# anuradhawick/kmertools

Hardware: AMD Instinct MI355X
Metric: Gbases/s on comp-oligo k=4 and ctr k=31, 150bp synthetic reads, 1/2/4/8 GPU (higher is better)
Workload: dtype f64

## Files before the change

kmertools_amd/csrc/kt_bulk.hip:

```cpp
#include <stdio.h>
#include <stdlib.h>

#include <new>
#include <type_traits>
#include <vector>

#include "kt_launch.hpp"
#include "kt_segment.hpp"
#include "kt_superkmer.hpp"
#include "kt_table.hpp"

namespace {

using ktseg::SegArgs;
using ktseg::SegShared;
using kttab::Slot;
using kttab::TableRef;

constexpr int BLOCK = ktseg::BLOCK;
#ifndef KT_BUILD_T
#define KT_BUILD_T 1024
#endif
#ifndef KT_ABLATION
#define KT_ABLATION 0
#endif
constexpr uint32_t LOG2_S = kttab::LOG2_RANGE;
constexpr uint32_t S = 1u << LOG2_S;
constexpr uint32_t MAX_B = 2048;
#ifndef KT_STORE_HASH
#define KT_STORE_HASH 1
#endif
#ifndef KT_P2_BIG32_PER
#define KT_P2_BIG32_PER 16
#endif
#ifndef KT_P2_T64
#define KT_P2_T64 512
#endif
template <class K, bool BIG>
constexpr int p2t() { return BIG ? (sizeof(K) == 8 ? KT_P2_T64 : 1024) : 512; }
template <class K, bool BIG>
constexpr bool p2_sdig() { return !BIG && !(sizeof(K) == 8 && KT_STORE_HASH); }
template <class K, bool BIG>
constexpr uint32_t chunk2() { return sizeof(K) == 8 ? (BIG ? 16384u : 8192u) : (BIG ? (uint32_t)KT_P2_BIG32_PER : 32u) * p2t<K, BIG>(); }

struct Plan {
    uint32_t n;
    uint32_t m8;
    uint32_t b1, b2;
    uint32_t B1, B2;
    uint32_t G;
    uint64_t cap1;
    uint64_t cap2;
    uint64_t room1;
    uint32_t nxs, xmap;
    uint32_t dbg;
    uint32_t lists;
    uint32_t kbits;
};

template <class K>
constexpr K empty_of() { return (K) ~(K)0; }

struct Meta {
    uint32_t *H;
    uint64_t *O;
    uint64_t *bstart;
    uint64_t *gcur;
    unsigned long long *dump;
    unsigned long long *xcur;
    uint32_t *ovf;
    kt_seg_src *srcs;
    uint32_t *fail;
    uint64_t *fstart;
    uint64_t *fend;
    uint64_t *spill_n;
    uint64_t *spill_keys;
    uint32_t *spill_counts;
    uint64_t spill_cap;
};

__device__ __forceinline__ uint32_t digit1h(uint64_t h, const Plan &p) { return (uint32_t)(h >> 32) >> (32 - p.b1); }
__device__ __forceinline__ uint32_t digit2h(uint64_t h, const Plan &p) {
    return ((uint32_t)(h >> 32) >> (32 - p.b1 - p.b2)) & (p.B2 - 1);
}
__device__ __forceinline__ uint32_t digit1(uint64_t key, const Plan &p) { return digit1h(ktd::khash_k(key, p.kbits), p); }
static_assert(KT_KHASH == 1 || !KT_STORE_HASH,
              "the empty marker must not be the hash of a k-mer (true for the multiplicative hash)");
template <class K>
constexpr bool stores_hash() { return sizeof(K) == 8 && KT_STORE_HASH; }
template <class K>
// ... 1485 lines not shown
            for (uint32_t i = tid; i < B2; i += P2T) {
                fstart[(uint64_t)jl * B2 + i] = lo + (uint64_t)i * cap2;
                fend[(uint64_t)jl * B2 + i] = lo + sm.cur[i];
            }
        } else if (tid == 0) {
            fail[jl] = 1u;
            atomicAdd(&fail[p.B1], 1u);
        }
        ktd::lds_barrier();
    }
}

template <class K>
struct SwwcShared {
    K *buf;
    uint32_t *fc;
    uint32_t *flags;
    static size_t bytes(uint32_t B2) { return (size_t)B2 * 128 + (size_t)B2 * 8 + 64; }
    __device__ SwwcShared(unsigned char *raw, uint32_t B2) {
        buf = reinterpret_cast<K *>(raw);
        fc = reinterpret_cast<uint32_t *>(raw + (size_t)B2 * 128);
        flags = fc + 2 * B2;
    }
};
#ifndef KT_SWWC_T64
#define KT_SWWC_T64 1024
#endif
#ifndef KT_SWWC_T32
#define KT_SWWC_T32 1024
#endif
template <class K>
constexpr int swwc_t() { return sizeof(K) == 8 ? KT_SWWC_T64 : KT_SWWC_T32; }

template <class K>
__global__ __launch_bounds__((swwc_t<K>()), (swwc_t<K>() / 256)) void part2_swwc_kernel(P2In in, Plan p, K *__restrict__ keys2,
                                                              uint64_t *__restrict__ fstart, uint64_t *__restrict__ fend,
                                                              uint32_t *__restrict__ fail) {
    extern __shared__ __attribute__((aligned(16))) unsigned char smem_raw[];
    const SwwcShared<K> sm(smem_raw, p.B2);
    constexpr K EMPTY = empty_of<K>();
#ifndef KT_SWWC_PER32
#define KT_SWWC_PER32 16
#endif
#ifndef KT_SWWC_PER64
#define KT_SWWC_PER64 8
#endif
    constexpr int P2T = swwc_t<K>(), PER = sizeof(K) == 8 ? KT_SWWC_PER64 : KT_SWWC_PER32 * 512 / P2T;
    constexpr uint32_t CH = (uint32_t)P2T * PER;
    constexpr uint32_t LK = 128 / sizeof(K), LSH = sizeof(K) == 8 ? 4 : 5;
    constexpr uint32_t GL = 8;
    constexpr uint32_t KPL = LK / GL;
    const uint32_t tid = threadIdx.x;
    const uint32_t nd = p.B1;
    const uint32_t B2 = p.B2, cap2 = (uint32_t)p.cap2, dshift = 32 - p.b1 - p.b2;
    auto digit = [&](K stored) -> uint32_t { return ((uint32_t)(hash_of_stored<K>(stored, p) >> 32) >> dshift) & (B2 - 1u); };
    const uint32_t grp = tid / GL, gl = tid % GL;
    for (uint32_t jl = blockIdx.x; jl < nd; jl += gridDim.x) {
        const uint32_t n_seg = in.n_src;
        auto segment = [&](uint32_t sidx, const K *&base, uint64_t &n) {
            const kt_seg_src &q = in.srcs[sidx];
            const uint64_t c = q.counts[jl];
            base = reinterpret_cast<const K *>(q.keys) + (uint64_t)jl * q.cap1;
            n = c < q.cap1 ? c : q.cap1;
        };
        uint64_t total = 0;
        for (uint32_t sidx = 0; sidx < n_seg; sidx++) {
            const K *b;
            uint64_t n;
            segment(sidx, b, n);
            total += n;
        }
        if (fail[jl] != 0) continue;
        const uint64_t lo = in.out_of(jl, p.room1);
        for (uint32_t i = tid; i < 2 * B2; i += P2T) sm.fc[i] = 0;
        if (tid < 4) sm.flags[tid] = 0;
        ktd::lds_barrier();
        const kt_i32x4 outrs = buf_rsrc(keys2 + lo, (uint32_t)(p.room1 * sizeof(K)));
        const uint32_t allow_a = (uint32_t)__builtin_amdgcn_readfirstlane(
            (int)__float_as_uint(0.93f * (float)cap2 / (float)(total ? total : 1)));
        const uint32_t allow_b = (uint32_t)__builtin_amdgcn_readfirstlane((int)__float_as_uint(6.f * sqrtf((float)cap2) + 32.f));
        uint64_t seen = 0;
        bool failed = false;
        K kcur[PER], knext[PER];
        uint32_t qa[PER];
#ifndef KT_SWWC_FB
#define KT_SWWC_FB 4
#endif
        auto flush = [&](uint32_t g, float allowed) {
            constexpr uint32_t FB = KT_SWWC_FB, NGR = P2T / GL;
            for (uint32_t d0 = 0; d0 < B2; d0 += NGR * FB) {
                uint32_t fl[FB], cu[FB];
                bool some = false;
#pragma unroll
                for (uint32_t b = 0; b < FB; b++) {
                    const uint32_t d = d0 + b * NGR + grp;
                    fl[b] = d < B2 ? sm.fc[2 * d] : 0u;
                    cu[b] = d < B2 ? sm.fc[2 * d + 1] : 0u;
                }
#pragma unroll
                for (uint32_t b = 0; b < FB; b++) some |= (fl[b] >> LSH) != 0;
                typedef uint32_t raw4 __attribute__((ext_vector_type(4)));
                raw4 v[FB];
#pragma unroll
                for (uint32_t b = 0; b < FB; b++) v[b] = raw4{0u, 0u, 0u, 0u};
                if (__builtin_amdgcn_ballot_w64(some) != 0) {
#pragma unroll
                    for (uint32_t b = 0; b < FB; b++) {
                        const uint32_t d = d0 + b * NGR + grp;
                        v[b] = *reinterpret_cast<const raw4 *>(&sm.buf[(size_t)(d < B2 ? d : 0) * LK + gl * KPL]);
                    }
                }
#pragma unroll
                for (uint32_t b = 0; b < FB; b++) {
                    const uint32_t d = d0 + b * NGR + grp;
                    if (d0 + b * NGR >= B2) break;
                    const uint32_t fill = fl[b], cur = cu[b];
                    const bool go = (fill >> LSH) != 0;
                    const bool fits = cur + LK <= cap2;
                    const uint32_t off = go && fits ? (d * cap2 + cur + gl * KPL) * (uint32_t)sizeof(K) : BUF_DROP;
                    asm volatile("buffer_store_dwordx4 %0, %1, %2, 0 offen\n\ts_nop 1" ::"v"(v[b]), "v"(off), "s"(outrs));
                    if (go && gl == 0) {
                        sm.fc[2 * d] = fill - LK;
                        sm.fc[2 * d + 1] = cur + LK;
                        if ((fill >> LSH) > 1) sm.flags[(g + 1) & 1] = 1;
                        if (!fits || (float)(cur + fill) > allowed) sm.flags[2] = 1;
                    }
                }
            }
        };
        for (uint32_t sidx = 0; sidx < n_seg && !failed; sidx++) {
            const K *base;
            uint64_t n;
            segment(sidx, base, n);
            if (n == 0) continue;
            auto load_chunk = [&](uint64_t c0, K (&dst)[PER]) {
                const uint32_t left = (uint32_t)__builtin_amdgcn_readfirstlane((int)(n - c0 > CH ? CH : (uint32_t)(n - c0)));
                const kt_i32x4 rs = buf_rsrc(base + c0, left * (uint32_t)sizeof(K));
                uint32_t voff = tid * (uint32_t)sizeof(K);
#pragma unroll
                for (int u = 0; u < PER; u += 8) buf_load8_async<K, P2T * (int)sizeof(K)>(&dst[u], rs, voff);
            };
            load_chunk(0, knext);
            buf_take<0>(kcur, knext);
            for (uint64_t c0 = 0; c0 < n; c0 += CH) {
                uint32_t tl = tid;
                asm volatile("" : "+v"(tl));
                const uint32_t left = (uint32_t)__builtin_amdgcn_readfirstlane((int)(n - c0 > CH ? CH : (uint32_t)(n - c0)));
                if (left != CH) {
#pragma unroll
                    for (int u = 0; u < PER; u++) kcur[u] = (uint32_t)u * P2T + tl < left ? kcur[u] : EMPTY;
                }
                const bool more = c0 + CH < n;
                if (more) load_chunk(c0 + CH, knext);
                if (tl == 0) sm.flags[0] = 0;
#pragma unroll
                for (int u = 0; u < PER; u++) {
                    const uint32_t d = digit(kcur[u]);
                    const bool valid = kcur[u] != EMPTY;
                    const uint32_t q = atomicAdd(&sm.fc[2 * d], valid ? 1u : 0u);
                    qa[u] = valid ? ((q >> LSH) << 16) | (d * LK + (q & (LK - 1u))) : ~0u;
                }
                ktd::lds_barrier();
                if (sm.flags[2] != 0) {
                    failed = true;
                    if (more) buf_drain(knext);
                    break;
                }
                const uint64_t sn = seen + c0 + CH;
                const float allowed = (float)(uint32_t)(sn < total ? sn : total) * __uint_as_float(allow_a) + __uint_as_float(allow_b);
#pragma unroll
                for (int u = 0; u < PER; u++)
                    if ((qa[u] >> 16) == 0u) sm.buf[qa[u] & 0xFFFFu] = kcur[u];
                for (uint32_t i = tl; i < B2; i += P2T)
                    if ((sm.fc[2 * i] >> LSH) != 0) sm.flags[0] = 1;
                if (tl == 0) sm.flags[1] = 0;
                ktd::lds_barrier();
                bool any = sm.flags[0] != 0;
                uint32_t gens = 0;
                for (uint32_t g = 0; any; g++) {
                    flush(g, allowed);
                    gens++;
                    ktd::lds_barrier();
                    any = sm.flags[(g + 1) & 1] != 0;
                    if (tl == 0) sm.flags[g & 1] = 0;
#pragma unroll
                    for (int u = 0; u < PER; u++)
                        if ((qa[u] >> 16) == g + 1u) sm.buf[qa[u] & 0xFFFFu] = kcur[u];
                    if (any) ktd::lds_barrier();
                }
                if (more) {
                    constexpr int SPG = (1024 + P2T / GL - 1) / (P2T / GL);
                    const uint32_t issued = gens * ((B2 + P2T / GL - 1) / (P2T / GL));
                    if (issued == SPG) buf_take<SPG>(kcur, knext);
                    else if (issued == 2 * SPG) buf_take<2 * SPG>(kcur, knext);
                    else if (issued == 3 * SPG) buf_take<3 * SPG>(kcur, knext);
                    else buf_take<0>(kcur, knext);
                }
            }
            seen += n;
        }
        ktd::lds_barrier();
        if (!failed) {
            for (uint32_t d0 = 0; d0 < B2; d0 += P2T / GL) {
                const uint32_t d = d0 + grp;
                if (d >= B2) continue;
                const uint32_t fill = sm.fc[2 * d], cur = sm.fc[2 * d + 1];
                if (cur + fill > cap2) {
                    sm.flags[2] = 1;
                    continue;
                }
                for (uint32_t e = gl * KPL; e < gl * KPL + KPL; e++)
                    if (e < fill) keys2[lo + (uint64_t)d * cap2 + cur + e] = sm.buf[(size_t)d * LK + e];
                if (gl == 0) {
                    fstart[(uint64_t)jl * B2 + d] = lo + (uint64_t)d * cap2;
                    fend[(uint64_t)jl * B2 + d] = lo + (uint64_t)d * cap2 + cur + fill;
                }
            }
        }
        ktd::lds_barrier();
        if ((failed || sm.flags[2] != 0) && tid == 0) {
            fail[jl] = 1u;
            atomicAdd(&fail[p.B1], 1u);
        }
        ktd::lds_barrier();
    }
}

static_assert(LOG2_S == kttab::LOG2_RANGE, "a fine bucket is a range of the table");

constexpr int BUILD_T = KT_BUILD_T;
constexpr uint32_t LIST_CAP = 192, LIST_KEYS = LIST_CAP * (BUILD_T / 64);

template <class K>
struct lds_word;
template <>
struct lds_word<uint64_t> { using type = unsigned long long; };
template <>
struct lds_word<uint32_t> { using type = unsigned int; };

constexpr uint32_t XBLK = 8192;
static_assert(XBLK >= (1u << LOG2_S), "a range's entries fit one block");
struct ExtOut {
    uint64_t *keys;
    uint32_t *counts;
    uint64_t max;
    uint64_t *ovf_keys;
    uint32_t *ovf_counts;
    uint64_t ovf_cap;
    uint64_t *extent;
    uint32_t *fill;
    uint64_t max_blocks;
    __device__ __forceinline__ void put(uint64_t pos, uint64_t key, uint32_t occ) const {
        if (pos < max) {
            __builtin_nontemporal_store(key, keys + pos);
            __builtin_nontemporal_store(occ, counts + pos);
        } else if (pos - max < ovf_cap) {
            ovf_keys[pos - max] = key;
            ovf_counts[pos - max] = occ;
        }
    }
    __device__ __forceinline__ void get(uint64_t pos, uint64_t &key, uint32_t &occ) const {
        if (pos < max) {
            key = keys[pos];
            occ = counts[pos];
        } else {
            key = ovf_keys[pos - max];
            occ = ovf_counts[pos - max];
        }
    }
};

#ifndef KT_BUILD_DHASH
#define KT_BUILD_DHASH 1
#endif
#ifndef KT_BUILD_SGPRS
#define KT_BUILD_SGPRS 80
#endif
template <class K, bool MERGE, bool DENSE, bool EXT = false, bool DIRECT = false>
__global__ __launch_bounds__(BUILD_T) __attribute__((amdgpu_num_sgpr(KT_BUILD_SGPRS), amdgpu_waves_per_eu(8, 8))) void build_kernel(const K *__restrict__ keys2,
                                                        const uint64_t *__restrict__ fstart,
                                                        const uint64_t *__restrict__ fend, Plan p,
                                                        Slot *__restrict__ slots, uint64_t *__restrict__ spill_n,
                                                        uint64_t *__restrict__ spill_keys,
                                                        uint32_t *__restrict__ spill_counts, uint64_t spill_cap,
                                                        uint32_t *__restrict__ spill_ovf,
                                                        uint64_t *__restrict__ distinct,
                                                        uint32_t *__restrict__ range_counts, ExtOut xo) {
    static_assert(!(MERGE && DENSE), "a dense build starts from an empty table");
    static_assert(!EXT || DENSE, "only a dense build writes to the export arrays");
    static_assert(!DIRECT || (DENSE && sizeof(K) == 4), "the direct build: 32-bit keys, dense");
    extern __shared__ __attribute__((aligned(16))) unsigned char smem_raw[];
    using W = typename lds_word<K>::type;
    constexpr K EMPTY = empty_of<K>();
    const uint32_t RS = p.m8 << (LOG2_S - 3);
    K *const skeys = reinterpret_cast<K *>(smem_raw);
    uint32_t *const scounts = reinterpret_cast<uint32_t *>(smem_raw + (size_t)RS * sizeof(K));
    const uint32_t tid = threadIdx.x, lane = tid & 63u;
    const uint64_t n_fine = (uint64_t)(p.B1) * p.B2;
    const uint32_t shift = 64 - p.n;
    auto spill = [&](uint64_t key, uint32_t occurrences) {
        if (DENSE) {
            atomicOr(spill_ovf, 1u);
            return;
        }
        const uint64_t at = atomicAdd(reinterpret_cast<unsigned long long *>(spill_n), 1ull);
        if (at < spill_cap) {
            spill_keys[at] = key;
            spill_counts[at] = occurrences;
        } else {
            atomicOr(spill_ovf, 1u);
        }
    };
    __shared__ uint32_t runs[BUILD_T / 64];
    uint16_t *const mylist = reinterpret_cast<uint16_t *>(smem_raw + (size_t)RS * (sizeof(K) + 4)) + (threadIdx.x >> 6) * LIST_CAP;
    bool dirty = true;
    uint64_t xpos = 0, xend = 0;
    uint32_t xused = 0;
    long long placed = 0;
    uint64_t lo = 0, hi = 0;
    K head[4] = {EMPTY, EMPTY, EMPTY, EMPTY};
    auto load_head = [&](uint64_t l, uint64_t h, K (&dst)[4]) {
#pragma unroll
        for (int u = 0; u < 4; u++) {
            const uint64_t i = l + tid + (uint64_t)u * BUILD_T;
            dst[u] = i < h ? keys2[i] : EMPTY;
        }
    };
    if (blockIdx.x < n_fine) {
        lo = fstart[blockIdx.x];
        hi = fend[blockIdx.x];
        load_head(lo, hi, head);
    }
#if KT_ABLATION
    unsigned long long tph = __builtin_readcyclecounter();
    uint32_t phs[8] = {};
#endif
    for (uint64_t fb = blockIdx.x; fb < n_fine;) {
        const uint64_t nfb = fb + gridDim.x;
        uint64_t nlo = 0, nhi = 0;
        if (nfb < n_fine) {
            nlo = fstart[nfb];
            nhi = fend[nfb];
        }
        if (MERGE && lo == hi) {
            fb = nfb;
            lo = nlo;
            hi = nhi;
            load_head(lo, hi, head);
            continue;
        }
        if (MERGE) {
            for (uint32_t i = tid; i < RS; i += BUILD_T) {
                const uint4 v = reinterpret_cast<const uint4 *>(slots + fb * RS)[i];
                const bool occ = (v.x & v.y) != 0xFFFFFFFFu;
                skeys[i] = occ ? to_stored<K>(((uint64_t)v.y << 32) | v.x) : EMPTY;
                scounts[i] = v.z;
                placed -= occ;
            }
        } else if (dirty) {
            for (uint32_t i = tid; i < RS; i += BUILD_T) {
                if (!DIRECT) skeys[i] = EMPTY;
                scounts[i] = 0;
            }
        }
        const bool listed = !DIRECT && DENSE && p.lists != 0 && hi - lo <= LIST_KEYS && hi - lo <= RS;
        KT_PH(0);
        if (MERGE || dirty) ktd::lds_barrier();
        KT_PH(1);
        uint32_t wc = 0;
        uint32_t m0 = ~0u, m1 = ~0u;
        if constexpr (DIRECT) {
            const uint32_t sh32 = 32u - p.kbits;
            auto bump = [&](K key) {
                if (key != EMPTY) atomicAdd(&scounts[ktd::nhash((uint32_t)key, p.kbits) & (S - 1u)], 1u);
            };
            (void)sh32;
            uint64_t bbase = lo;
            for (;;) {
                const bool more = bbase + 4ull * BUILD_T < hi;
                K nxt[4] = {EMPTY, EMPTY, EMPTY, EMPTY};
                if (more) load_head(bbase + 4ull * BUILD_T, hi, nxt);
#pragma unroll
                for (int u = 0; u < 4; u++) bump(head[u]);
                if (!more) break;
                bbase += 4ull * BUILD_T;
#pragma unroll
                for (int u = 0; u < 4; u++) head[u] = nxt[u];
            }
        } else {
            constexpr bool STRIDES = KT_BUILD_DHASH && DENSE && sizeof(K) == 8;
            const uint32_t sh3 = shift - 3;
            auto hword = [&](K stored, auto hi_only) -> uint32_t {
                const uint64_t h = hash_of_stored<K>(stored, p);
                const uint32_t hi32 = (uint32_t)(h >> 32), lo32 = (uint32_t)h;
                if constexpr (decltype(hi_only)::value) return hi32 >> (sh3 - 32);
                else return __builtin_amdgcn_alignbit(hi32, lo32, sh3);
            };
            auto home_w = [&](uint32_t w) -> uint32_t { return __umul24((w >> 3) & (S - 1), p.m8) >> 3; };
            auto stride_w = [&](uint32_t w) -> uint32_t {
                if (!STRIDES) return 1u;
                return __builtin_amdgcn_perm(0x251f1d17u, 0x13110d0bu, (w & 7u) | 0x0c0c0c00u);
            };
            auto insert_batch = [&](auto chk, auto lst, auto hi_only) {
                constexpr bool CHECK = decltype(chk)::value, LISTED = decltype(lst)::value;
                K cur = head[0], q0 = head[1], q1 = head[2], q2 = LISTED ? EMPTY : head[3];
#if KT_ABLATION
                if (p.dbg & 1u) cur = EMPTY;
#endif
                uint32_t w = hword(cur, hi_only);
                uint32_t s = home_w(w), step = stride_w(w), probes = 0;
                while (cur != EMPTY) {
                    const K v = (K)atomicCAS(reinterpret_cast<W *>(&skeys[s]), (W)EMPTY, (W)cur);
                    const bool claimed = v == EMPTY, dup = v == cur;
                    bool done = claimed | dup;
                    if (dup) atomicAdd(&scounts[s], 1u);
                    if constexpr (LISTED) {
                        if (claimed) {
                            m1 = __builtin_amdgcn_alignbit(m1, m0, 16);
                            m0 = (m0 << 16) | s;
                        }
                    }
                    s += step;
                    if (s >= RS) s -= RS;
                    if (CHECK && !done && ++probes >= RS) {
                        spill(from_stored<K>(cur), 1u);
                        done = true;
                    }
                    if (done) {
                        cur = q0;
                        q0 = q1;
                        q1 = q2;
                        q2 = EMPTY;
                        w = hword(cur, hi_only);
                        s = home_w(w);
                        step = stride_w(w);
                        if (CHECK) probes = 0;
                    }
                }
            };
            const bool roomy = !MERGE && hi - lo <= RS;
            uint64_t bbase = lo;
            for (;;) {
                const bool more = bbase + 4ull * BUILD_T < hi;
                K nxt[4] = {EMPTY, EMPTY, EMPTY, EMPTY};
                if (more) load_head(bbase + 4ull * BUILD_T, hi, nxt);
                auto insert = [&](auto hi_only) {
                    if (listed) insert_batch(std::false_type{}, std::true_type{}, hi_only);
                    else if (roomy) insert_batch(std::false_type{}, std::false_type{}, hi_only);
                    else insert_batch(std::true_type{}, std::false_type{}, hi_only);
                };
                if (sh3 >= 32) insert(std::true_type{});
                else insert(std::false_type{});
                if (!more) break;
                bbase += 4ull * BUILD_T;
#pragma unroll
                for (int u = 0; u < 4; u++) head[u] = nxt[u];
            }
        }
        if (DENSE && listed) {
            const uint32_t c = (uint32_t)((m0 & 0xFFFFu) != 0xFFFFu) + (uint32_t)((m0 >> 16) != 0xFFFFu) +
                               (uint32_t)((m1 & 0xFFFFu) != 0xFFFFu);
            const uint32_t inc = wave_incl_scan(c);
            uint16_t *const at = mylist + (inc - c);
            if (c > 0) at[0] = (uint16_t)m0;
            if (c > 1) at[1] = (uint16_t)(m0 >> 16);
            if (c > 2) at[2] = (uint16_t)m1;
            wc = (uint32_t)__builtin_amdgcn_readlane((int)inc, 63);
            if (lane == 0) runs[tid >> 6] = wc;
        }
        KT_PH(2);
        ktd::lds_barrier();
        KT_PH(3);
        load_head(nlo, nhi, head);
        uint4 *dst = reinterpret_cast<uint4 *>(slots + fb * RS);
        if (DENSE) {
            constexpr uint32_t NW = BUILD_T / 64;
            const uint32_t wave = tid >> 6, share = RS / NW;
            if (!listed) {
                for (uint32_t i0 = 0; i0 < share; i0 += 64) {
                    const uint32_t i = wave * share + i0 + lane;
                    K kk;
                    uint32_t cc;
                    if constexpr (DIRECT) {
                        const uint32_t c1 = scounts[i];
                        cc = c1 - 1u;
                        kk = c1 ? (K)ktd::nhash_inv(((uint32_t)fb << LOG2_S) | i, p.kbits) : EMPTY;
                    } else {
                        kk = skeys[i];
                        cc = scounts[i];
                    }
                    const uint64_t bal = __ballot(kk != EMPTY);
                    if (kk != EMPTY) {
                        const uint32_t at = wave * share + wc + (uint32_t)__popcll(bal & ((1ull << lane) - 1ull));
                        skeys[at] = kk;
                        scounts[at] = cc;
                    }
                    wc += (uint32_t)__popcll(bal);
                }
                if (lane == 0) runs[wave] = wc;
                KT_PH(4);
                ktd::lds_barrier();
                KT_PH(5);
            }
            auto take = [&](uint32_t e, K &kk, uint32_t &cc) {
                const uint32_t src = listed ? (uint32_t)mylist[e] : wave * share + e;
                kk = skeys[src];
// ... 72 lines not shown
                        __builtin_nontemporal_store(cc, dcounts + pre + (j - skew));
                    }
                }
                if (tid == 0) {
                    range_counts[fb] = D;
                    placed += D;
                }
            }
#if KT_ABLATION
        } else if (!(p.dbg & 8u)) {
#else
        } else {
#endif
            for (uint32_t i = tid; i < RS; i += BUILD_T) {
                const K kk = skeys[i];
                const uint64_t key = kk == EMPTY ? KT_EMPTY_KEY : from_stored<K>(kk);
                placed += kk != EMPTY;
#if KT_BUILD_NT
                typedef uint32_t raw4 __attribute__((ext_vector_type(4)));
                const raw4 raw = {(uint32_t)key, (uint32_t)(key >> 32), scounts[i], 0u};
                __builtin_nontemporal_store(raw, reinterpret_cast<raw4 *>(dst + i));
#else
                dst[i] = make_uint4((uint32_t)key, (uint32_t)(key >> 32), scounts[i], 0u);
#endif
            }
        }
        dirty = !listed;
        KT_PH(6);
        ktd::lds_barrier();
        KT_PH(7);
        fb = nfb;
        lo = nlo;
        hi = nhi;
    }
#if KT_ABLATION
    if (tid == 0)
        for (int i = 0; i < 8; i++) atomicAdd(&kt_dbg_phase[i], (unsigned long long)phs[i]);
#endif
    if (EXT && tid == 0 && xend) {
        if (xend / XBLK - 1 < xo.max_blocks) xo.fill[xend / XBLK - 1] = XBLK - (uint32_t)(xend - xpos);
        atomicMax(reinterpret_cast<unsigned long long *>(xo.extent), (unsigned long long)xend);
    }
    for (int o = 32; o > 0; o >>= 1) placed += __shfl_down(placed, o, 64);
    if (lane == 0 && placed) atomicAdd(reinterpret_cast<unsigned long long *>(distinct), (unsigned long long)placed);
}

constexpr uint32_t XSCAN_WGS = 32, XSCAN_CH = 1024 * 16;
__device__ __forceinline__ uint64_t ext_holes_before(const uint64_t *__restrict__ hpre, const uint64_t *__restrict__ info,
                                                     uint64_t j) {
    return hpre[j] + info[8 + (j >> info[4])];
}
__global__ __launch_bounds__(1024) void ext_scan_kernel(ExtOut xo, uint64_t *__restrict__ hpre, uint64_t max_blocks,
                                                         uint64_t patch_grid, uint64_t *__restrict__ info,
                                                         uint32_t *__restrict__ flags) {
    __shared__ uint64_t wtot[16];
    __shared__ uint64_t carry;
    __shared__ bool last;
    const uint64_t T = *xo.extent;
    uint64_t nb = T / XBLK;
    const bool too_far = nb > max_blocks || (T > xo.max && T - xo.max > xo.ovf_cap);
    if (too_far) {
        if (threadIdx.x == 0 && blockIdx.x == 0) {
            atomicOr(flags, 4u);
            info[0] = info[1] = info[2] = info[3] = 0;
        }
        return;
// ... 302 lines not shown
        }
    }
}

uint64_t env_u64(const char *name, uint64_t dflt) {
    const char *s = getenv(name);
    if (!s || !*s) return dflt;
    return strtoull(s, nullptr, 10);
}

}

enum SourceKind { SRC_READS, SRC_KEYS, SRC_RECORDS, SRC_PACKED };
struct SourceRec {
    SourceKind kind;
    ReadsSource rs;
    KeysSource ks;
    RecordSource rc;
    PackedSource ps;
    uint64_t n_units;
};
template <class F>
static int with_source(const SourceRec &r, F &&f) {
    switch (r.kind) {
        case SRC_READS: return f(r.rs);
        case SRC_KEYS: return f(r.ks);
        case SRC_PACKED: return f(r.ps);
        default: return f(r.rc);
    }
}

struct BulkKnobs {
    uint64_t bulk, min_bases, merge_div, g_mult, paged, fixed2, p2_big64, p2_big32, build_wgs, dense,
        verbose, ext_ovf_blocks, build_wgs_ext, direct, pack, p2_fast, p2_grid, p2_swwc, b1, build_lists, s1y;
};
static BulkKnobs read_knobs() {
    BulkKnobs k;
    k.bulk = env_u64("KT_BULK", 1);
    k.min_bases = env_u64("KT_BULK_MIN_BASES", 4ull << 20);
    k.merge_div = env_u64("KT_BULK_MERGE_DIV", 8);
    k.g_mult = env_u64("KT_BULK_G_MULT", 1);
    k.paged = env_u64("KT_BULK_PAGED", 1);
    k.fixed2 = env_u64("KT_BULK_FIXED2", 1);
    k.s1y = env_u64("KT_S1Y", 1);
    k.p2_big64 = env_u64("KT_P2_BIG64", 1);
    k.p2_big32 = env_u64("KT_P2_BIG32", 0);
    k.p2_grid = env_u64("KT_P2_GRID", 0);
    k.b1 = env_u64("KT_BULK_B1", 0);
    k.p2_swwc = env_u64("KT_P2_SWWC", 1);
    k.p2_fast = env_u64("KT_P2_FAST", 1);
    k.build_wgs = env_u64("KT_BUILD_WGS", 64);
    k.build_wgs_ext = env_u64("KT_BUILD_WGS_EXT", 16);
    k.build_lists = env_u64("KT_BUILD_LISTS", 1);
    k.dense = env_u64("KT_BULK_DENSE", 1);
    k.direct = env_u64("KT_BUILD_DIRECT", 1);
    k.pack = env_u64("KT_BULK_PACK", 1);
    k.verbose = env_u64("KT_BULK_VERBOSE", 0);
    k.ext_ovf_blocks = env_u64("KT_EXT_OVF_BLOCKS", 0);
    return k;
}

struct kt_bulk_job {
    Plan p{};
    BulkKnobs kn{};
    Meta m{};
    bool narrow = false;
    bool paged = false, merge = false, open = false;
    bool xcd = false;
    uint64_t max_keys = 0, added_bound = 0;
    std::vector<SourceRec> srcs;
    kt_seg_src p2_src{};
    size_t desc_used = 0;
    std::vector<std::vector<uint64_t>> desc_host;
    size_t ksz() const { return narrow ? 4 : 8; }
};

void kt_bulk_job_free(kt_bulk_job *job) { delete job; }

namespace {

template <class K>
int level1_paged(kt_ctr *ctr, kt_bulk_job &j, const SourceRec &r) {
    kt_ctx *ctx = ctr->ctx;
    K *keys1 = (K *)ctr->b_keys1.p;
    if (!j.xcd) return kt::fail(KT_ERR_ARG, "bulk build: paged level 1 without its cursors");
    unsigned long long *xcur = j.m.xcur;
    const Plan p = j.p;
    uint32_t *const ovf = j.m.ovf;
    unsigned long long *const dump = j.m.dump;
    const bool two = j.kn.s1y && Scatter1YShared<K, 1024>::bytes(j.p.B1) <= 160 * 1024;
    const uint32_t mult = (uint32_t)(j.kn.g_mult ? j.kn.g_mult : 1);
    const uint32_t cus = (uint32_t)ctx->n_cu > 2 * ctr->l1_spare_cus ? (uint32_t)ctx->n_cu - ctr->l1_spare_cus : (uint32_t)ctx->n_cu;
    return with_source(r, [&](const auto &src) -> int {
        using S = std::decay_t<decltype(src)>;
        if (two) {
            constexpr int T = 1024;
            const size_t lds = Scatter1YShared<K, T>::bytes(p.B1);
            auto kern = scatter1y_kernel<S, K, T>;
            KT_HIP(hipFuncSetAttribute(reinterpret_cast<const void *>(kern), hipFuncAttributeMaxDynamicSharedMemorySize, (int)lds));
            hipLaunchKernelGGL(kern, dim3(cus * mult), dim3(T), lds, ctx->stream, src, p, xcur, ovf, keys1, dump);
// ... 40 lines not shown
    return KT_OK;
}

template <class K>
int finish_typed(kt_ctr *ctr, kt_bulk_job &j) {
    kt_ctx *ctx = ctr->ctx;
    Plan &p = j.p;
    Meta &m = j.m;
    K *keys1 = (K *)ctr->b_keys1.p, *keys2 = (K *)ctr->b_keys2.p;
    if (j.paged) {
        hipLaunchKernelGGL(xcd_tails_kernel<K>, dim3(p.B1), dim3(BLOCK), 0, ctx->stream, p, (const unsigned long long *)m.xcur, m.gcur, keys1);
        uint32_t ovf = 0;
        KT_HIP(hipMemcpyAsync(&ovf, m.ovf, 4, hipMemcpyDeviceToHost, ctx->stream));
        KT_HIP(hipStreamSynchronize(ctx->stream));
        if (ovf) {
            j.paged = false;
            ctr->paged_failed = true;
            p.cap1 = 0;
            p.cap2 = 0;
            if (j.added_bound > ctr->b_keys1.cap / sizeof(K)) {
                return kt::fail(KT_ERR_NOMEM, "bulk build: key buffers too small for the exact layout");
            }
            if (int rc = level1_exact<K>(ctr, j)) return rc;
        }
    }
    P2In in{keys1, m.bstart, nullptr, 0};
    if (j.paged) {
        j.p2_src = kt_seg_src{keys1, m.gcur, p.cap1};
        KT_HIP(hipMemcpyAsync(m.srcs, &j.p2_src, sizeof(kt_seg_src), hipMemcpyHostToDevice, ctx->stream));
        in.srcs = m.srcs;
        in.n_src = 1;
    }
    const uint32_t nd = p.B1;
    auto run_part2 = [&](const Plan &pp, const P2In &src, K *out, uint64_t *fs, uint64_t *fe, uint32_t *fail) -> int {
        if (pp.cap2 && src.srcs && j.kn.p2_swwc && pp.B2 >= 512 && SwwcShared<K>::bytes(pp.B2) <= 160 * 1024) {
            const size_t lds = SwwcShared<K>::bytes(pp.B2);
            KT_HIP(hipMemsetAsync(fail, 0, ((size_t)pp.B1 + 1) * 4, ctx->stream));
            auto swwc = part2_swwc_kernel<K>;
            KT_HIP(hipFuncSetAttribute(reinterpret_cast<const void *>(swwc), hipFuncAttributeMaxDynamicSharedMemorySize, (int)lds));
            uint32_t grid = pp.B1;
            if (j.kn.p2_grid && grid > j.kn.p2_grid) grid = (uint32_t)j.kn.p2_grid;
            hipLaunchKernelGGL(swwc, dim3(grid), dim3(swwc_t<K>()), lds, ctx->stream, src, pp, out, fs, fe, fail);
            KT_HIP(hipGetLastError());
            const bool bigr = (sizeof(K) == 8 ? j.kn.p2_big64 : j.kn.p2_big32) != 0 && Part2Shared<K, true>::bytes(pp.B2) <= 160 * 1024;
            auto redo_launch = [&](auto big) -> int {
                constexpr bool BIG = decltype(big)::value;
                const size_t rl = Part2Shared<K, BIG>::bytes(pp.B2);
                auto redo = part2_kernel<K, false, BIG>;
                KT_HIP(hipFuncSetAttribute(reinterpret_cast<const void *>(redo), hipFuncAttributeMaxDynamicSharedMemorySize, (int)rl));
                hipLaunchKernelGGL(redo, dim3(pp.B1), dim3(p2t<K, BIG>()), rl, ctx->stream, src, pp, out, fs, fe,
                                   (const uint32_t *)fail);
                KT_HIP(hipGetLastError());
                return KT_OK;
            };
            return bigr ? redo_launch(std::true_type{}) : redo_launch(std::false_type{});
        }
        const bool big2 = (sizeof(K) == 8 ? j.kn.p2_big64 : j.kn.p2_big32) != 0 &&
                          Part2Shared<K, true>::bytes(pp.B2) <= 160 * 1024;
        auto launch = [&](auto big) -> int {
            constexpr bool BIG = decltype(big)::value;
            const size_t part2_lds = Part2Shared<K, BIG>::bytes(pp.B2);
            constexpr uint32_t P2T = (uint32_t)p2t<K, BIG>();
            if (pp.cap2 && src.srcs && j.kn.p2_fast && pp.B2 <= 4 * P2T) {
                KT_HIP(hipMemsetAsync(fail, 0, ((size_t)pp.B1 + 1) * 4, ctx->stream));
                auto go = [&](auto pb) -> int {
                    constexpr int PB = decltype(pb)::value;
                    auto fast = part2_fast_kernel<K, BIG, PB>;
                    KT_HIP(hipFuncSetAttribute(reinterpret_cast<const void *>(fast), hipFuncAttributeMaxDynamicSharedMemorySize,
                                               (int)part2_lds));
                    uint32_t grid = pp.B1;
                    if (j.kn.p2_grid && grid > j.kn.p2_grid) grid = (uint32_t)j.kn.p2_grid;
                    hipLaunchKernelGGL(fast, dim3(grid), dim3(P2T), part2_lds, ctx->stream, src, pp, out, fs, fe, fail);
                    KT_HIP(hipGetLastError());
                    return KT_OK;
                };
                const int rc = pp.B2 <= P2T       ? go(std::integral_constant<int, 1>{})
                               : pp.B2 <= 2 * P2T ? go(std::integral_constant<int, 2>{})
                                                  : go(std::integral_constant<int, 4>{});
                if (rc) return rc;
                auto redo = part2_kernel<K, false, BIG>;
                KT_HIP(hipFuncSetAttribute(reinterpret_cast<const void *>(redo), hipFuncAttributeMaxDynamicSharedMemorySize,
                                           (int)part2_lds));
                hipLaunchKernelGGL(redo, dim3(pp.B1), dim3(P2T), part2_lds, ctx->stream, src, pp, out, fs, fe,
                                   (const uint32_t *)fail);
                KT_HIP(hipGetLastError());
                return KT_OK;
            }
            const bool l16 = KT_P2_LOAD16 && sizeof(K) == 8 && pp.cap2 && src.srcs;
            auto part2 = !pp.cap2 ? part2_kernel<K, false, BIG> : l16 ? part2_kernel<K, true, BIG, true> : part2_kernel<K, true, BIG>;
            KT_HIP(hipFuncSetAttribute(reinterpret_cast<const void *>(part2), hipFuncAttributeMaxDynamicSharedMemorySize,
                                       (int)part2_lds));
            hipLaunchKernelGGL(part2, dim3(pp.B1), dim3(P2T), part2_lds, ctx->stream, src, pp, out, fs, fe,
                               (const uint32_t *)nullptr);
            KT_HIP(hipGetLastError());
            return KT_OK;
        };
        return big2 ? launch(std::true_type{}) : launch(std::false_type{});
    };
    if (int rc = run_part2(p, in, keys2, m.fstart, m.fend, m.fail)) return rc;
    const uint64_t n_fine = (uint64_t)nd * p.B2;
    const bool dense = !j.merge && j.kn.dense != 0;
    bool ext = dense && ctr->xt_keys && ctr->xt_counts;
    uint64_t gb = (uint64_t)ctx->n_cu * (ext ? j.kn.build_wgs_ext : j.kn.build_wgs);
    if (gb > n_fine) gb = n_fine;
    size_t build_lds = (size_t)(p.m8 << (LOG2_S - 3)) * (sizeof(K) + 4);
    p.lists = dense && j.kn.build_lists && build_lds + LIST_KEYS * 2 + 256 <= 80 * 1024 ? 1u : 0u;
    if (p.lists) build_lds += LIST_KEYS * 2;
    auto launch_build = [&](bool to_ext, const ExtOut &xo) -> int {
        auto build = j.merge ? build_kernel<K, true, false>
                     : to_ext ? build_kernel<K, false, true, true>
                     : dense  ? build_kernel<K, false, true>
                              : build_kernel<K, false, false>;
        if constexpr (sizeof(K) == 4) {
            if (dense && !j.merge && j.kn.direct && p.kbits && p.n == p.kbits && p.m8 == 8)
                build = to_ext ? build_kernel<K, false, true, true, true> : build_kernel<K, false, true, false, true>;
        }
        KT_HIP(hipFuncSetAttribute(reinterpret_cast<const void *>(build), hipFuncAttributeMaxDynamicSharedMemorySize,
                                   (int)build_lds));
        hipLaunchKernelGGL(build, dim3((uint32_t)gb), dim3(BUILD_T), build_lds, ctx->stream, (const K *)keys2, m.fstart,
                           m.fend, p, (Slot *)ctr->slots, m.spill_n, m.spill_keys, m.spill_counts, m.spill_cap, ctr->flags,
                           ctr->distinct, ctr->range_counts, xo);
        KT_HIP(hipGetLastError());
        return KT_OK;
    };
    if (ext) {
        const uint64_t ovf_cap = (j.kn.ext_ovf_blocks ? j.kn.ext_ovf_blocks - 1 : 2 * gb + 2) * XBLK;
        const uint64_t max_blocks = (ctr->xt_max + ovf_cap) / XBLK + 2;
        size_t off = 0;
        const size_t off_fill = off;  off += (max_blocks * 4 + 255) & ~(size_t)255;
        const size_t off_hpre = off;  off += ((max_blocks + 1) * 8 + 255) & ~(size_t)255;
        const size_t off_info = off;  off += ((8 + XSCAN_WGS + 1) * 8 + 255) & ~(size_t)255;
        const size_t off_ok = off;    off += (ovf_cap * 8 + 255) & ~(size_t)255;
        const size_t off_oc = off;    off += (ovf_cap * 4 + 255) & ~(size_t)255;
        if (int rc = ctr->b_ext.reserve(off)) return rc;
        char *xb = (char *)ctr->b_ext.p;
        uint64_t *hpre = (uint64_t *)(xb + off_hpre), *xinfo = (uint64_t *)(xb + off_info);
        const ExtOut xo{ctr->xt_keys, ctr->xt_counts, ctr->xt_max, (uint64_t *)(xb + off_ok), (uint32_t *)(xb + off_oc),
                        ovf_cap,      ctr->cursor,    (uint32_t *)(xb + off_fill), max_blocks};
        KT_HIP(hipMemsetAsync(ctr->cursor, 0, 8, ctx->stream));
        KT_HIP(hipMemsetAsync(xo.fill, 0, max_blocks * 4, ctx->stream));
        if (int rc = launch_build(true, xo)) return rc;
        const uint64_t patch_grid = ovf_cap / XBLK + 3;
        KT_HIP(hipMemsetAsync(xinfo, 0, (8 + XSCAN_WGS + 1) * 8, ctx->stream));
        hipLaunchKernelGGL(ext_scan_kernel, dim3(XSCAN_WGS), dim3(1024), 0, ctx->stream, xo, hpre, max_blocks, patch_grid, xinfo, ctr->flags);
        hipLaunchKernelGGL(ext_patch_kernel, dim3((uint32_t)patch_grid), dim3(256), 0, ctx->stream, xo,
                           (const uint64_t *)hpre, (const uint64_t *)xinfo, (const uint32_t *)ctr->flags);
        KT_HIP(hipGetLastError());
        uint32_t fl = 0, l2_redone = 0;
        KT_HIP(hipMemcpyAsync(&fl, ctr->flags, 4, hipMemcpyDeviceToHost, ctx->stream));
        KT_HIP(hipMemcpyAsync(&l2_redone, m.fail + p.B1, 4, hipMemcpyDeviceToHost, ctx->stream));
        KT_HIP(hipStreamSynchronize(ctx->stream));
        ctr->l2_redone = l2_redone;
        ctr->l2_buckets = p.B1;
        if (fl & 6u) {
            if (fl & 2u) ctr->xt_too_small = true;
            fl &= ~6u;
            KT_HIP(hipMemcpyAsync(ctr->flags, &fl, 4, hipMemcpyHostToDevice, ctx->stream));
            KT_HIP(hipMemsetAsync(ctr->distinct, 0, 8, ctx->stream));
            KT_HIP(hipStreamSynchronize(ctx->stream));
            ext = false;
            if (j.kn.verbose) fprintf(stderr, "[bulk] export-target build redone into the table (%s)\n",
                                      ctr->xt_too_small ? "arrays too small" : "uneven blocks");
        }
    }
    if (!ext)
        if (int rc = launch_build(false, ExtOut{})) return rc;
    ctr->dense = dense;
    ctr->dense_ext = ext;
    if (!dense) {
        TableRef t{(Slot *)ctr->slots, ktl::geom_of(ctr), ctr->flags};
        hipLaunchKernelGGL(spill_insert_kernel, dim3(ctx->n_cu), dim3(BLOCK), 0, ctx->stream, m.spill_n, m.spill_keys,
                           m.spill_counts, m.spill_cap, t, ctr->distinct);
    }
    KT_HIP(hipGetLastError());
    if (j.kn.verbose) {
        uint64_t spilled = 0;
        KT_HIP(hipMemcpyAsync(&spilled, m.spill_n, 8, hipMemcpyDeviceToHost, ctx->stream));
        KT_HIP(hipStreamSynchronize(ctx->stream));
        fprintf(stderr, "[bulk] k=%d keys<=%llu level1=%s level2=%s %s spilled=%llu\n", ctr->k,
                (unsigned long long)j.max_keys, j.paged ? "paged" : "exact", p.cap2 ? "fixed" : "exact",
                j.merge ? "merge" : "build", (unsigned long long)spilled);
    }
    return KT_OK;
}

}

static int xcc_sets(kt_ctx *ctx, uint32_t *nxs, uint32_t *xmap) {
    if (!ctx->xcc_n) {
        if (int rc = ctx->s_aux2.reserve(256)) return rc;
        uint32_t *mask = (uint32_t *)ctx->s_aux2.p, h = 0;
        KT_HIP(hipMemsetAsync(mask, 0, 4, ctx->stream));
        hipLaunchKernelGGL(xcc_census_kernel, dim3((uint32_t)ctx->n_cu * 4), dim3(64), 0, ctx->stream, mask);
        KT_HIP(hipGetLastError());
        KT_HIP(hipMemcpyAsync(&h, mask, 4, hipMemcpyDeviceToHost, ctx->stream));
        KT_HIP(hipStreamSynchronize(ctx->stream));
        if (!(h & 0xFFu)) h = 1;
        uint32_t n = 0, map = 0;
        for (uint32_t id = 0; id < 8; id++)
            if (h >> id & 1u) map |= (n++) << (4 * id);
        ctx->xcc_n = n;
        ctx->xcc_map = map;
    }
    uint32_t b = 0;
    while ((1u << b) < ctx->xcc_n) b++;
    if (const char *e = getenv("KT_S1X_SETS")) {
        const uint32_t want = (uint32_t)atoi(e);
        uint32_t wb = 0;
        while ((1u << wb) < want && wb < 3) wb++;
        if (wb < b) {
            uint32_t map = 0;
            for (uint32_t id = 0; id < 8; id++) map |= (((ctx->xcc_map >> (4 * id)) & 7u) & ((1u << wb) - 1u)) << (4 * id);
            *nxs = wb;
            *xmap = map;
// ... 380 lines not shown
```

Before: 757.6.

## Store level-2 partitioned 32-bit keys as 16-bit hash indices for direct build

In the direct dense build, the software write-combining partition pass now replaces each key with its 16-bit counter index (top hash bits) and writes 64 keys per 128-byte line, half the bytes of full 32-bit keys. The build kernel reads these 16-bit values and bumps counters directly, so it no longer re-hashes. Ranges that failed the fixed-capacity pass and were redone fall back to the wide 32-bit form, detected through the fail array. This lowers global memory traffic between the two passes, at the cost of extra template variants and more complex cursor and offset arithmetic.

```diff
diff --git a/kmertools_amd/csrc/kt_bulk.hip b/kmertools_amd/csrc/kt_bulk.hip
--- a/kmertools_amd/csrc/kt_bulk.hip
+++ b/kmertools_amd/csrc/kt_bulk.hip
@@ -7,6 +7,7 @@
 
 #include "kt_launch.hpp"
 #include "kt_segment.hpp"
+#include "kt_short.hpp"
 #include "kt_superkmer.hpp"
 #include "kt_table.hpp"
 
@@ -56,6 +57,7 @@
     uint32_t dbg;
     uint32_t lists;
     uint32_t kbits;
+    uint32_t shortf;
 };
 
 template <class K>
@@ -1607,7 +1609,7 @@
 template <class K>
 constexpr int swwc_t() { return sizeof(K) == 8 ? KT_SWWC_T64 : KT_SWWC_T32; }
 
-template <class K>
+template <class K, bool SHORT = false>
 __global__ __launch_bounds__((swwc_t<K>()), (swwc_t<K>() / 256)) void part2_swwc_kernel(P2In in, Plan p, K *__restrict__ keys2,
                                                               uint64_t *__restrict__ fstart, uint64_t *__restrict__ fend,
                                                               uint32_t *__restrict__ fail) {
@@ -1622,9 +1624,21 @@
 #endif
     constexpr int P2T = swwc_t<K>(), PER = sizeof(K) == 8 ? KT_SWWC_PER64 : KT_SWWC_PER32 * 512 / P2T;
     constexpr uint32_t CH = (uint32_t)P2T * PER;
-    constexpr uint32_t LK = 128 / sizeof(K), LSH = sizeof(K) == 8 ? 4 : 5;
+    static_assert(!SHORT || sizeof(K) == 4, "the short form: 16 bits of a 32-bit key's hash");
+    constexpr uint32_t LK = SHORT ? ktshort::LK16 : 128 / sizeof(K);
+    constexpr uint32_t SL = LK;
+    constexpr uint32_t CUR1 = SHORT ? 1u : LK;
     constexpr uint32_t GL = 8;
-    constexpr uint32_t KPL = LK / GL;
+    static_assert((uint64_t)1024 * SL <= 65536, "a slot number fits 16 bits");
+    auto cur_keys = [&](uint32_t cur) -> uint32_t { return SHORT ? cur * LK : cur; };
+    auto cur_bytes = [&](uint32_t cur) -> uint32_t { return SHORT ? cur * 128u : cur * (uint32_t)sizeof(K); };
+    auto put = [&](uint32_t slot, K key) {
+        if constexpr (!SHORT) {
+            sm.buf[slot] = key;
+        } else {
+            reinterpret_cast<uint16_t *>(smem_raw)[slot] = (uint16_t)key;
+        }
+    };
     const uint32_t tid = threadIdx.x;
     const uint32_t nd = p.B1;
     const uint32_t B2 = p.B2, cap2 = (uint32_t)p.cap2, dshift = 32 - p.b1 - p.b2;
@@ -1673,7 +1687,7 @@
                     cu[b] = d < B2 ? sm.fc[2 * d + 1] : 0u;
                 }
 #pragma unroll
-                for (uint32_t b = 0; b < FB; b++) some |= (fl[b] >> LSH) != 0;
+                for (uint32_t b = 0; b < FB; b++) some |= fl[b] >= LK;
                 typedef uint32_t raw4 __attribute__((ext_vector_type(4)));
                 raw4 v[FB];
 #pragma unroll
@@ -1682,7 +1696,7 @@
 #pragma unroll
                     for (uint32_t b = 0; b < FB; b++) {
                         const uint32_t d = d0 + b * NGR + grp;
-                        v[b] = *reinterpret_cast<const raw4 *>(&sm.buf[(size_t)(d < B2 ? d : 0) * LK + gl * KPL]);
+                        v[b] = *reinterpret_cast<const raw4 *>(smem_raw + (size_t)(d < B2 ? d : 0) * 128 + gl * 16);
                     }
                 }
 #pragma unroll
@@ -1690,15 +1704,15 @@
                     const uint32_t d = d0 + b * NGR + grp;
                     if (d0 + b * NGR >= B2) break;
                     const uint32_t fill = fl[b], cur = cu[b];
-                    const bool go = (fill >> LSH) != 0;
-                    const bool fits = cur + LK <= cap2;
-                    const uint32_t off = go && fits ? (d * cap2 + cur + gl * KPL) * (uint32_t)sizeof(K) : BUF_DROP;
+                    const bool go = fill >= LK;
+                    const bool fits = cur_keys(cur) + LK <= cap2;
+                    const uint32_t off = go && fits ? d * cap2 * (uint32_t)sizeof(K) + cur_bytes(cur) + gl * 16u : BUF_DROP;
                     asm volatile("buffer_store_dwordx4 %0, %1, %2, 0 offen\n\ts_nop 1" ::"v"(v[b]), "v"(off), "s"(outrs));
                     if (go && gl == 0) {
                         sm.fc[2 * d] = fill - LK;
-                        sm.fc[2 * d + 1] = cur + LK;
-                        if ((fill >> LSH) > 1) sm.flags[(g + 1) & 1] = 1;
-                        if (!fits || (float)(cur + fill) > allowed) sm.flags[2] = 1;
+                        sm.fc[2 * d + 1] = cur + CUR1;
+                        if (fill >= 2 * LK) sm.flags[(g + 1) & 1] = 1;
+                        if (!fits || (float)(cur_keys(cur) + fill) > allowed) sm.flags[2] = 1;
                     }
                 }
             }
@@ -1733,7 +1747,10 @@
                     const uint32_t d = digit(kcur[u]);
                     const bool valid = kcur[u] != EMPTY;
                     const uint32_t q = atomicAdd(&sm.fc[2 * d], valid ? 1u : 0u);
-                    qa[u] = valid ? ((q >> LSH) << 16) | (d * LK + (q & (LK - 1u))) : ~0u;
+                    const uint32_t gen = q / LK;
+                    qa[u] = valid ? (gen << 16) | (d * SL + (q - gen * LK)) : ~0u;
+                    if constexpr (SHORT)
+                        kcur[u] = (K)((ktd::nhash_top((uint32_t)kcur[u], p.kbits) >> (32u - p.kbits)) & (S - 1u));
                 }
                 ktd::lds_barrier();
                 if (sm.flags[2] != 0) {
@@ -1745,9 +1762,9 @@
                 const float allowed = (float)(uint32_t)(sn < total ? sn : total) * __uint_as_float(allow_a) + __uint_as_float(allow_b);
 #pragma unroll
                 for (int u = 0; u < PER; u++)
-                    if ((qa[u] >> 16) == 0u) sm.buf[qa[u] & 0xFFFFu] = kcur[u];
+                    if ((qa[u] >> 16) == 0u) put(qa[u] & 0xFFFFu, kcur[u]);
                 for (uint32_t i = tl; i < B2; i += P2T)
-                    if ((sm.fc[2 * i] >> LSH) != 0) sm.flags[0] = 1;
+                    if (sm.fc[2 * i] >= LK) sm.flags[0] = 1;
                 if (tl == 0) sm.flags[1] = 0;
                 ktd::lds_barrier();
                 bool any = sm.flags[0] != 0;
@@ -1760,7 +1777,7 @@
                     if (tl == 0) sm.flags[g & 1] = 0;
 #pragma unroll
                     for (int u = 0; u < PER; u++)
-                        if ((qa[u] >> 16) == g + 1u) sm.buf[qa[u] & 0xFFFFu] = kcur[u];
+                        if ((qa[u] >> 16) == g + 1u) put(qa[u] & 0xFFFFu, kcur[u]);
                     if (any) ktd::lds_barrier();
                 }
                 if (more) {
@@ -1779,13 +1796,22 @@
             for (uint32_t d0 = 0; d0 < B2; d0 += P2T / GL) {
                 const uint32_t d = d0 + grp;
                 if (d >= B2) continue;
-                const uint32_t fill = sm.fc[2 * d], cur = sm.fc[2 * d + 1];
+                const uint32_t fill = sm.fc[2 * d], cur = cur_keys(sm.fc[2 * d + 1]);
                 if (cur + fill > cap2) {
                     sm.flags[2] = 1;
                     continue;
                 }
-                for (uint32_t e = gl * KPL; e < gl * KPL + KPL; e++)
-                    if (e < fill) keys2[lo + (uint64_t)d * cap2 + cur + e] = sm.buf[(size_t)d * LK + e];
+                if constexpr (SHORT) {
+                    typedef uint32_t raw4 __attribute__((ext_vector_type(4)));
+                    unsigned char *const region = reinterpret_cast<unsigned char *>(keys2 + lo + (uint64_t)d * cap2);
+                    if (gl * 16u < fill * 2u)
+                        *reinterpret_cast<raw4 *>(region + (size_t)cur_bytes(sm.fc[2 * d + 1]) + gl * 16) =
+                            *reinterpret_cast<const raw4 *>(smem_raw + (size_t)d * 128 + gl * 16);
+                } else {
+                    constexpr uint32_t KPL = LK / GL;
+                    for (uint32_t e = gl * KPL; e < gl * KPL + KPL; e++)
+                        if (e < fill) keys2[lo + (uint64_t)d * cap2 + cur + e] = sm.buf[(size_t)d * LK + e];
+                }
                 if (gl == 0) {
                     fstart[(uint64_t)jl * B2 + d] = lo + (uint64_t)d * cap2;
                     fend[(uint64_t)jl * B2 + d] = lo + (uint64_t)d * cap2 + cur + fill;
@@ -1851,7 +1877,7 @@
 #ifndef KT_BUILD_SGPRS
 #define KT_BUILD_SGPRS 80
 #endif
-template <class K, bool MERGE, bool DENSE, bool EXT = false, bool DIRECT = false>
+template <class K, bool MERGE, bool DENSE, bool EXT = false, bool DIRECT = false, bool SHORT = false>
 __global__ __launch_bounds__(BUILD_T) __attribute__((amdgpu_num_sgpr(KT_BUILD_SGPRS), amdgpu_waves_per_eu(8, 8))) void build_kernel(const K *__restrict__ keys2,
                                                         const uint64_t *__restrict__ fstart,
                                                         const uint64_t *__restrict__ fend, Plan p,
@@ -1860,8 +1886,10 @@
                                                         uint32_t *__restrict__ spill_counts, uint64_t spill_cap,
                                                         uint32_t *__restrict__ spill_ovf,
                                                         uint64_t *__restrict__ distinct,
-                                                        uint32_t *__restrict__ range_counts, ExtOut xo) {
+                                                        uint32_t *__restrict__ range_counts, ExtOut xo,
+                                                        const uint32_t *__restrict__ fail) {
     static_assert(!(MERGE && DENSE), "a dense build starts from an empty table");
+    static_assert(!SHORT || DIRECT, "the short form: the direct build's counter indices");
     static_assert(!EXT || DENSE, "only a dense build writes to the export arrays");
     static_assert(!DIRECT || (DENSE && sizeof(K) == 4), "the direct build: 32-bit keys, dense");
     extern __shared__ __attribute__((aligned(16))) unsigned char smem_raw[];
@@ -1894,17 +1922,33 @@
     long long placed = 0;
     uint64_t lo = 0, hi = 0;
     K head[4] = {EMPTY, EMPTY, EMPTY, EMPTY};
-    auto load_head = [&](uint64_t l, uint64_t h, K (&dst)[4]) {
+    auto range_wide = [&](uint64_t f) -> bool {
+        if constexpr (SHORT) return __builtin_amdgcn_readfirstlane((int)fail[f >> p.b2]) != 0;
+        else return true;
+    };
+    auto load_head = [&](bool wide, uint64_t base, uint64_t l, uint64_t h, K (&dst)[4]) {
+        (void)wide; (void)base;
 #pragma unroll
         for (int u = 0; u < 4; u++) {
             const uint64_t i = l + tid + (uint64_t)u * BUILD_T;
-            dst[u] = i < h ? keys2[i] : EMPTY;
+            if constexpr (SHORT) {
+                if (wide) {
+                    const K key = i < h ? keys2[i] : EMPTY;
+                    dst[u] = key != EMPTY ? (K)(ktd::nhash((uint32_t)key, p.kbits) & (S - 1u)) : EMPTY;
+                } else {
+                    dst[u] = i < h ? (K) reinterpret_cast<const uint16_t *>(keys2 + base)[i - base] : EMPTY;
+                }
+            } else {
+                dst[u] = i < h ? keys2[i] : EMPTY;
+            }
         }
     };
+    bool wide = true, nwide = true;
     if (blockIdx.x < n_fine) {
         lo = fstart[blockIdx.x];
         hi = fend[blockIdx.x];
-        load_head(lo, hi, head);
+        wide = range_wide(blockIdx.x);
+        load_head(wide, lo, lo, hi, head);
     }
 #if KT_ABLATION
     unsigned long long tph = __builtin_readcyclecounter();
@@ -1916,12 +1960,13 @@
         if (nfb < n_fine) {
             nlo = fstart[nfb];
             nhi = fend[nfb];
+            nwide = range_wide(nfb);
         }
         if (MERGE && lo == hi) {
             fb = nfb;
             lo = nlo;
             hi = nhi;
-            load_head(lo, hi, head);
+            load_head(true, lo, lo, hi, head);
             continue;
         }
         if (MERGE) {
@@ -1945,16 +1990,18 @@
         uint32_t wc = 0;
         uint32_t m0 = ~0u, m1 = ~0u;
         if constexpr (DIRECT) {
-            const uint32_t sh32 = 32u - p.kbits;
             auto bump = [&](K key) {
-                if (key != EMPTY) atomicAdd(&scounts[ktd::nhash((uint32_t)key, p.kbits) & (S - 1u)], 1u);
+                if constexpr (SHORT) {
+                    if (key != EMPTY) atomicAdd(&scounts[key], 1u);
+                } else {
+                    if (key != EMPTY) atomicAdd(&scounts[ktd::nhash((uint32_t)key, p.kbits) & (S - 1u)], 1u);
+                }
             };
-            (void)sh32;
             uint64_t bbase = lo;
             for (;;) {
                 const bool more = bbase + 4ull * BUILD_T < hi;
                 K nxt[4] = {EMPTY, EMPTY, EMPTY, EMPTY};
-                if (more) load_head(bbase + 4ull * BUILD_T, hi, nxt);
+                if (more) load_head(wide, lo, bbase + 4ull * BUILD_T, hi, nxt);
 #pragma unroll
                 for (int u = 0; u < 4; u++) bump(head[u]);
                 if (!more) break;
@@ -2018,7 +2065,7 @@
             for (;;) {
                 const bool more = bbase + 4ull * BUILD_T < hi;
                 K nxt[4] = {EMPTY, EMPTY, EMPTY, EMPTY};
-                if (more) load_head(bbase + 4ull * BUILD_T, hi, nxt);
+                if (more) load_head(wide, lo, bbase + 4ull * BUILD_T, hi, nxt);
                 auto insert = [&](auto hi_only) {
                     if (listed) insert_batch(std::false_type{}, std::true_type{}, hi_only);
                     else if (roomy) insert_batch(std::false_type{}, std::false_type{}, hi_only);
@@ -2046,7 +2093,7 @@
         KT_PH(2);
         ktd::lds_barrier();
         KT_PH(3);
-        load_head(nlo, nhi, head);
+        load_head(nwide, nlo, nlo, nhi, head);
         uint4 *dst = reinterpret_cast<uint4 *>(slots + fb * RS);
         if (DENSE) {
             constexpr uint32_t NW = BUILD_T / 64;
@@ -2185,6 +2232,7 @@
         fb = nfb;
         lo = nlo;
         hi = nhi;
+        wide = nwide;
     }
 #if KT_ABLATION
     if (tid == 0)
@@ -2553,7 +2601,7 @@
 
 struct BulkKnobs {
     uint64_t bulk, min_bases, merge_div, g_mult, paged, fixed2, p2_big64, p2_big32, build_wgs, dense,
-        verbose, ext_ovf_blocks, build_wgs_ext, direct, pack, p2_fast, p2_grid, p2_swwc, b1, build_lists, s1y;
+        verbose, ext_ovf_blocks, build_wgs_ext, direct, pack, p2_fast, p2_grid, p2_swwc, p2_short, b1, build_lists, s1y;
 };
 static BulkKnobs read_knobs() {
     BulkKnobs k;
@@ -2569,6 +2617,7 @@
     k.p2_grid = env_u64("KT_P2_GRID", 0);
     k.b1 = env_u64("KT_BULK_B1", 0);
     k.p2_swwc = env_u64("KT_P2_SWWC", 1);
+    k.p2_short = env_u64("KT_P2_SHORT", 1);
     k.p2_fast = env_u64("KT_P2_FAST", 1);
     k.build_wgs = env_u64("KT_BUILD_WGS", 64);
     k.build_wgs_ext = env_u64("KT_BUILD_WGS_EXT", 16);
@@ -2587,6 +2636,7 @@
     Meta m{};
     bool narrow = false;
     bool paged = false, merge = false, open = false;
+    bool shortf = false;
     bool xcd = false;
     uint64_t max_keys = 0, added_bound = 0;
     std::vector<SourceRec> srcs;
@@ -2693,11 +2743,20 @@
         in.n_src = 1;
     }
     const uint32_t nd = p.B1;
+    auto takes_swwc = [&](const Plan &pp, const P2In &src) -> bool {
+        return pp.cap2 && src.srcs && j.kn.p2_swwc && pp.B2 >= 512 && SwwcShared<K>::bytes(pp.B2) <= 160 * 1024;
+    };
+    const bool dense = !j.merge && j.kn.dense != 0;
+    const bool direct = sizeof(K) == 4 && dense && j.kn.direct && p.kbits && p.n == p.kbits && p.m8 == 8;
+    j.shortf = j.kn.p2_short != 0 && direct && takes_swwc(p, in);
+    p.shortf = j.shortf ? 1u : 0u;
     auto run_part2 = [&](const Plan &pp, const P2In &src, K *out, uint64_t *fs, uint64_t *fe, uint32_t *fail) -> int {
-        if (pp.cap2 && src.srcs && j.kn.p2_swwc && pp.B2 >= 512 && SwwcShared<K>::bytes(pp.B2) <= 160 * 1024) {
+        if (takes_swwc(pp, src)) {
             const size_t lds = SwwcShared<K>::bytes(pp.B2);
             KT_HIP(hipMemsetAsync(fail, 0, ((size_t)pp.B1 + 1) * 4, ctx->stream));
-            auto swwc = part2_swwc_kernel<K>;
+            auto swwc = part2_swwc_kernel<K, false>;
+            if constexpr (sizeof(K) == 4)
+                if (pp.shortf) swwc = part2_swwc_kernel<K, true>;
             KT_HIP(hipFuncSetAttribute(reinterpret_cast<const void *>(swwc), hipFuncAttributeMaxDynamicSharedMemorySize, (int)lds));
             uint32_t grid = pp.B1;
             if (j.kn.p2_grid && grid > j.kn.p2_grid) grid = (uint32_t)j.kn.p2_grid;
@@ -2760,7 +2819,6 @@
     };
     if (int rc = run_part2(p, in, keys2, m.fstart, m.fend, m.fail)) return rc;
     const uint64_t n_fine = (uint64_t)nd * p.B2;
-    const bool dense = !j.merge && j.kn.dense != 0;
     bool ext = dense && ctr->xt_keys && ctr->xt_counts;
     uint64_t gb = (uint64_t)ctx->n_cu * (ext ? j.kn.build_wgs_ext : j.kn.build_wgs);
     if (gb > n_fine) gb = n_fine;
@@ -2773,14 +2831,16 @@
                      : dense  ? build_kernel<K, false, true>
                               : build_kernel<K, false, false>;
         if constexpr (sizeof(K) == 4) {
-            if (dense && !j.merge && j.kn.direct && p.kbits && p.n == p.kbits && p.m8 == 8)
-                build = to_ext ? build_kernel<K, false, true, true, true> : build_kernel<K, false, true, false, true>;
+            if (direct) {
+                build = j.shortf ? (to_ext ? build_kernel<K, false, true, true, true, true> : build_kernel<K, false, true, false, true, true>)
+                                 : (to_ext ? build_kernel<K, false, true, true, true> : build_kernel<K, false, true, false, true>);
+            }
         }
         KT_HIP(hipFuncSetAttribute(reinterpret_cast<const void *>(build), hipFuncAttributeMaxDynamicSharedMemorySize,
                                    (int)build_lds));
         hipLaunchKernelGGL(build, dim3((uint32_t)gb), dim3(BUILD_T), build_lds, ctx->stream, (const K *)keys2, m.fstart,
                            m.fend, p, (Slot *)ctr->slots, m.spill_n, m.spill_keys, m.spill_counts, m.spill_cap, ctr->flags,
-                           ctr->distinct, ctr->range_counts, xo);
+                           ctr->distinct, ctr->range_counts, xo, (const uint32_t *)m.fail);
         KT_HIP(hipGetLastError());
         return KT_OK;
     };
@@ -2836,11 +2896,14 @@
     KT_HIP(hipGetLastError());
     if (j.kn.verbose) {
         uint64_t spilled = 0;
+        uint32_t redone = 0;
         KT_HIP(hipMemcpyAsync(&spilled, m.spill_n, 8, hipMemcpyDeviceToHost, ctx->stream));
+        if (p.cap2 && in.srcs) KT_HIP(hipMemcpyAsync(&redone, m.fail + p.B1, 4, hipMemcpyDeviceToHost, ctx->stream));
         KT_HIP(hipStreamSynchronize(ctx->stream));
-        fprintf(stderr, "[bulk] k=%d keys<=%llu level1=%s level2=%s %s spilled=%llu\n", ctr->k,
+        fprintf(stderr, "[bulk] k=%d keys<=%llu level1=%s level2=%s %s spilled=%llu l2_redone=%u keys2=%s\n", ctr->k,
                 (unsigned long long)j.max_keys, j.paged ? "paged" : "exact", p.cap2 ? "fixed" : "exact",
-                j.merge ? "merge" : "build", (unsigned long long)spilled);
+                j.merge ? "merge" : "build", (unsigned long long)spilled, redone,
+                j.shortf ? "short16" : "wide");
     }
     return KT_OK;
 }
diff --git a/kmertools_amd/csrc/kt_short.hpp b/kmertools_amd/csrc/kt_short.hpp
--- /dev/null
+++ b/kmertools_amd/csrc/kt_short.hpp
@@ -0,0 +1,9 @@
+#pragma once
+#include <stdint.h>
+
+namespace ktshort {
+
+constexpr uint32_t LINE = 128;
+constexpr uint32_t LK16 = LINE / 2;
+
+}
```

After: 757.2. About the same (-0.0%).
